# yangt1013/SPEINet

Hardware: AMD Instinct MI355X
Metric: deblurred 720p frames/sec (higher is better)
Workload: dtype f16 (correlation top2)

## Files before the change

include/speinet_hip.h:

```cpp
#ifndef SPEINET_HIP_H
#define SPEINET_HIP_H

#include <stdint.h>

#ifdef __cplusplus
extern "C" {
#endif

typedef void* spei_stream_t;

#define SPEI_ACT_NONE 0
#define SPEI_ACT_RELU 1
#define SPEI_ACT_GELU 2

#define SPEI_F32 0
#define SPEI_BF16 1
#define SPEI_F16 2

#define SPEI_CONV 0
#define SPEI_CONV_TRANSPOSED 1

int spei_version(void);
const char* spei_last_error(void);
const char* spei_arch(void);

int spei_any_nonzero(const float* x, int64_t n, int32_t* flag, spei_stream_t stream);

int spei_rl_prior(const float* img, float* out, float* scratch, int C, int H, int W, int iters, float lam,
                  spei_stream_t stream);

int spei_conv5_in(const float* img_chw, const float* w, const float* bias, float* out_hwc, int H, int W,
                  int Cout, spei_stream_t stream);

int spei_conv5_out(const float* in_hwc, int ldi, const float* w, const float* bias, float* out_chw, int H,
                   int W, int Cin, spei_stream_t stream);

int spei_igemm_f32(const float* a0, int lda0, int k0, const float* a1, int lda1, int k1, const float* w,
                   const float* bias, float* out, int ldo, const float* residual, int ldr,
                   const float* rowscale, int Hin, int Win, int Hout, int Wout, int N, int ksize, int stride,
                   int pad, int mode, int act, spei_stream_t stream);

int spei_igemm_f32_batched(const float* a0, int lda0, int k0, const float* a1, int lda1, int k1, const float* w,
                           const float* bias, float* out, int ldo, const float* residual, int ldr,
                           const float* rowscale, int Hin, int Win, int Hout, int Wout, int N, int ksize, int stride,
                           int pad, int mode, int act, int batch, spei_stream_t stream);

int spei_igemm_bf16(const float* a0, int lda0, int k0, const float* a1, int lda1, int k1, const void* w_hi,
                    const void* w_lo, const float* bias, float* out, int ldo, const float* residual, int ldr,
                    const float* rowscale, int Hin, int Win, int Hout, int Wout, int N, int ksize, int stride,
                    int pad, int mode, int act, spei_stream_t stream);

int spei_conv_slab16(int fmt, const void* a0, int lda0, int k0, const void* a1, int lda1, int k1, int a_fmt,
                     const void* wfrag_hi, const void* wfrag_lo, const float* bias, void* out, int ldo, int out_fmt,
                     const float* residual, int ldr, const float* rowscale, int Hin, int Win, int Hout, int Wout,
                     int N, int ksize, int stride, int pad, int act, int ln_input, spei_stream_t stream);

int spei_conv_slab16_batched(int fmt, const void* a0, int k0, int a_fmt, const void* wfrag, const void* wfrag_lo, const float* bias,
                             void* out, int out_fmt, const float* residual, int batch, int Hin, int Win, int Hout, int Wout, int N,
                             int ksize, int stride, int pad, int act, spei_stream_t stream);

int spei_conv_slab16_fa(int fmt, const float* x, int K, const void* x1, const float* s, const float* g1, const float* g2,
                        float* x_out, const void* wfrag, const float* bias, void* out, int ldo, int out_fmt, int H, int W, int N,
                        int ksize, int act, spei_stream_t stream);

int spei_conv32_ws16(int fmt, const void* a, int a_fmt, const void* wfrag, const float* bias, void* out, int out_fmt, int batch,
                     int H, int W, int act, spei_stream_t stream);

int spei_mlp_fused16(int fmt, const float* x, float* out, const void* w1_frag, const float* b1, const void* w2_frag,
                     const float* b2, int64_t M, spei_stream_t stream);

int spei_convt2_slab16(int fmt, const void* a0, int lda0, int k0, int a_fmt, const void* wfrag00, const void* wfrag01,
                       const void* wfrag10, const void* wfrag11, const float* bias, void* out, int ldo, int out_fmt,
                       int Hin, int Win, int N, int act, spei_stream_t stream);

int spei_convt2_slab16x3(const float* a0, int lda0, int k0, const void* const* whi4, const void* const* wlo4, const float* bias,
                         float* out, int ldo, int Hin, int Win, int N, int act, spei_stream_t stream);

int spei_conv3x3_256_pipe16(int fmt, const float* x, const void* w_frag, const float* bias, const float* residual, float* out,
                            int batch, int H, int W, spei_stream_t stream);

int spei_conv5_out_slab16(int fmt, const void* in, int ldi, int in_fmt, const void* wfrag, const float* bias32, float* out_chw,
                          int H, int W, spei_stream_t stream);

int spei_attn_fused16(int fmt, const float* x, float* out, const void* yhat, const void* wq_frag, const float* bq,
                      const void* wkv_frag, const float* bkv, const void* wproj_frag, const float* bproj,
                      const float* relbias, int H, int W, int shift, spei_stream_t stream);

int spei_attn_win4_16(int fmt, const float* x, float* out, const void* yhat, const void* wq_frag, const float* bq,
                      const void* wkv_frag, const float* bkv, const void* wproj_frag, const float* bproj,
                      const float* relbias, int batch, int H, int W, int shift, spei_stream_t stream);

int64_t spei_frame_post_ws_doubles(int H, int W, int border);
int spei_frame_post(const float* out_chw, const unsigned char* gt_hwc, unsigned char* out_hwc, int H, int W, int border,
                    double* ws, double* result, spei_stream_t stream);

int64_t spei_gate_ws_floats(int H, int W, int C);
int spei_resblock_gates(const void* x1, int x1_fmt, int H, int W, int C, const float* se_w1, const float* se_b1,
                        const float* se_w2, const float* se_b2, const float* cw_w, const float* cw_bn,
                        const float* hc_w, const float* hc_bn, float* s, float* g1, float* g2, float* ws,
                        spei_stream_t stream);
int spei_resblock_apply(const float* x, const void* x1, int x1_fmt, const float* s, const float* g1, const float* g2,
                        const float* extra, float* out, int ldo, int H, int W, int C, spei_stream_t stream);

int spei_resblock_gates_batched(const void* x1, int x1_fmt, int batch, int H, int W, int C, const float* se_w1, const float* se_b1,
                                const float* se_w2, const float* se_b2, const float* cw_w, const float* cw_bn, const float* hc_w,
                                const float* hc_bn, float* s, float* g1, float* g2, float* ws, spei_stream_t stream);
int spei_resblock_apply_batched(const float* x, const void* x1, int x1_fmt, const float* s, const float* g1, const float* g2, float* out,
                                int batch, int H, int W, int C, spei_stream_t stream);

int spei_layernorm256(const float* x, void* y, int out_fmt, const float* gamma, const float* beta, int64_t M,
                      spei_stream_t stream);

int spei_window_attention(const void* q, const void* kv, int io_fmt, const float* relbias, void* out, int H, int W,
                          int shift, spei_stream_t stream);
int spei_window_attention_batched(const void* q, const void* kv, int io_fmt, const float* relbias, void* out, int H, int W,
                                  int shift, int batch, spei_stream_t stream);

int spei_patch_invnorm(const float* f, int ldf, float* inv, int H, int W, int C, spei_stream_t stream);

int64_t spei_corr_ws_floats(int64_t n_lr);
int spei_corr_argmax(const float* lr, int ldl, const float* ref, int ldr, const float* inv_lr,
                     const float* inv_ref, int Hl, int Wl, int Hr, int Wr, int C, float* S, int32_t* arg,
                     float* ws, spei_stream_t stream);

int spei_split16(int fmt, const float* x, int ld, void* hi, void* lo, int64_t M, int C, spei_stream_t stream);
int spei_corr_argmax_bf16(const void* lr_hi, const void* lr_lo, const void* ref_hi, const void* ref_lo,
                          const float* inv_lr, const float* inv_ref, int Hl, int Wl, int Hr, int Wr, int C, float* S,
                          int32_t* arg, float* ws, spei_stream_t stream);

int spei_corr_slab16(int fmt, const void* lr_hi, const void* lr_lo, const void* ref_hi, const void* ref_lo,
                     const float* inv_lr, const float* inv_ref, int Hl, int Wl, int Hr, int Wr, int C, float* S,
                     int32_t* arg, float* ws, spei_stream_t stream);

int spei_corr_slab_top2_16(int fmt, const void* lr16, const void* ref16, const float* inv_lr, const float* inv_ref,
                           int Hl, int Wl, int Hr, int Wr, int C, float* S, int32_t* arg, float* S2, int32_t* arg2,
                           float* ws, spei_stream_t stream);
int64_t spei_corr_diag_ws_floats(int Hl, int Wl, int Hr, int Wr);
int spei_corr_diag_top2_16(int fmt, const void* lr16, const void* ref16, const float* inv_ref, int Hl, int Wl, int Hr, int Wr,
                           int C, float* S, int32_t* arg, float* S2, int32_t* arg2, float* ws, spei_stream_t stream);
int spei_corr_rescore(const float* lr, int ldl, const float* ref, int ldr, const float* inv_lr, const float* inv_ref,
                      int Hl, int Wl, int Hr, int Wr, int C, float* S, int32_t* arg, const float* S2, const int32_t* arg2,
                      spei_stream_t stream);

int spei_gather_fold(const float* ref, int ldr, const int32_t* arg, float* out, int ldo, int H3, int W3,
                     int Hr3, int Wr3, int C, int s, spei_stream_t stream);

int spei_rot90(const float* in, int ldi, float* out, int H, int W, int C, spei_stream_t stream);

// ... 91 lines not shown
```

speinet_amd/_lib.py:

```python
from __future__ import annotations

import ctypes as C
import os
import re

_HERE = os.path.dirname(os.path.abspath(__file__))
LIB_PATH = os.path.join(_HERE, "libspeinet_hip.so")
HEADER_PATH = os.path.join(os.path.dirname(_HERE), "include", "speinet_hip.h")

_lib = None

P = C.c_void_p
I = C.c_int
L = C.c_int64
F = C.c_float

SIGNATURES = {
    "spei_version": (I, []),
    "spei_last_error": (C.c_char_p, []),
    "spei_arch": (C.c_char_p, []),
    "spei_any_nonzero": (I, [P, L, P, P]),
    "spei_rl_prior": (I, [P, P, P, I, I, I, I, F, P]),
    "spei_conv5_in": (I, [P, P, P, P, I, I, I, P]),
    "spei_conv5_out": (I, [P, I, P, P, P, I, I, I, P]),
    "spei_igemm_f32": (I, [P, I, I, P, I, I, P, P, P, I, P, I, P, I, I, I, I, I, I, I, I, I, I, P]),
    "spei_igemm_f32_batched": (I, [P, I, I, P, I, I, P, P, P, I, P, I, P, I, I, I, I, I, I, I, I, I, I, I, P]),
    "spei_igemm_bf16": (I, [P, I, I, P, I, I, P, P, P, P, I, P, I, P, I, I, I, I, I, I, I, I, I, I, P]),
    "spei_conv_slab16": (I, [I, P, I, I, P, I, I, I, P, P, P, P, I, I, P, I, P, I, I, I, I, I, I, I, I, I, I, P]),
    "spei_conv32_ws16": (I, [I, P, I, P, P, P, I, I, I, I, I, P]),
    "spei_conv_slab16_fa": (I, [I, P, I, P, P, P, P, P, P, P, P, I, I, I, I, I, I, I, P]),
    "spei_attn_fused16": (I, [I, P, P, P, P, P, P, P, P, P, P, I, I, I, P]),
    "spei_attn_win4_16": (I, [I, P, P, P, P, P, P, P, P, P, P, I, I, I, I, P]),
    "spei_conv5_out_slab16": (I, [I, P, I, I, P, P, P, I, I, P]),
    "spei_convt2_slab16": (I, [I, P, I, I, I, P, P, P, P, P, P, I, I, I, I, I, I, P]),
    "spei_convt2_slab16x3": (I, [P, I, I, P, P, P, P, I, I, I, I, I, P]),
    "spei_conv3x3_256_pipe16": (I, [I, P, P, P, P, P, I, I, I, P]),
    "spei_mlp_fused16": (I, [I, P, P, P, P, P, P, L, P]),
    "spei_split16": (I, [I, P, I, P, P, L, I, P]),
    "spei_corr_slab16": (I, [I, P, P, P, P, P, P, I, I, I, I, I, P, P, P, P]),
    "spei_corr_slab_top2_16": (I, [I, P, P, P, P, I, I, I, I, I, P, P, P, P, P, P]),
    "spei_pack_split16": (I, [P, I, I, I, I, P, P, P]),
    "spei_corr_diag_ws_floats": (L, [I, I, I, I]),
    "spei_corr_diag_top2_16": (I, [I, P, P, P, I, I, I, I, I, P, P, P, P, P, P]),
    "spei_corr_rescore": (I, [P, I, P, I, P, P, I, I, I, I, I, P, P, P, P, P]),
    "spei_corr_argmax_bf16": (I, [P, P, P, P, P, P, I, I, I, I, I, P, P, P, P]),
    "spei_gate_ws_floats": (L, [I, I, I]),
    "spei_resblock_gates": (I, [P, I, I, I, I, P, P, P, P, P, P, P, P, P, P, P, P, P]),
    "spei_resblock_apply": (I, [P, P, I, P, P, P, P, P, I, I, I, I, P]),
    "spei_resblock_apply_batched": (I, [P, P, I, P, P, P, P, I, I, I, I, P]),
    "spei_resblock_gates_batched": (I, [P, I, I, I, I, I, P, P, P, P, P, P, P, P, P, P, P, P, P]),
    "spei_conv_slab16_batched": (I, [I, P, I, I, P, P, P, P, I, P, I, I, I, I, I, I, I, I, I, I, P]),
    "spei_layernorm256": (I, [P, P, I, P, P, L, P]),
    "spei_window_attention": (I, [P, P, I, P, P, I, I, I, P]),
    "spei_window_attention_batched": (I, [P, P, I, P, P, I, I, I, I, P]),
    "spei_patch_invnorm": (I, [P, I, P, I, I, I, P]),
    "spei_corr_ws_floats": (L, [L]),
    "spei_corr_argmax": (I, [P, I, P, I, P, P, I, I, I, I, I, P, P, P, P]),
    "spei_gather_fold": (I, [P, I, P, P, I, I, I, I, I, I, I, P]),
    "spei_rot90": (I, [P, I, P, I, I, I, P]),
    "spei_upsample_bicubic": (I, [P, I, P, I, I, I, I, I, I, P]),
    "spei_add": (I, [P, P, P, L, P]),
    "spei_wgrad_ws_floats": (L, [I, I, I, I, I]),
    "spei_conv_wgrad_f32_batched": (I, [P, I, P, I, P, P, P, I, I, I, I, I, I, I, I, I, I, P]),
    "spei_conv_wgrad_bf16x3_batched": (I, [P, I, P, I, P, P, P, I, I, I, I, I, I, I, I, I, I, P]),
    "spei_conv_wgrad_bf16_batched": (I, [P, I, P, I, P, P, P, I, I, I, I, I, I, I, I, I, I, P]),
    "spei_conv_s2_adjoint_slab16": (I, [P, I, P, P, I, I, I, I, I, P]),
    "spei_conv_wgrad_f32": (I, [P, I, P, I, P, P, P, I, I, I, I, I, I, I, I, I, P]),
    "spei_relu_bwd": (I, [P, P, P, L, P]),
    "spei_plane_ws_floats": (L, [I, I, I]),
    "spei_plane_stats": (I, [P, P, I, I, I, I, P, P, P, P, P, P, P]),
    "spei_plane_stats_batched": (I, [P, P, I, I, I, I, P, P, P, P, P, P, I, P]),
    "spei_resblock_apply_bwd": (I, [P, P, P, P, P, P, P, P, P, P, P, P, P, I, I, I, P]),
    "spei_resblock_apply_bwd_batched": (I, [P, P, P, P, P, P, P, P, P, P, P, P, P, I, I, I, I, P]),
    "spei_gate_train_saved_floats": (L, [I, I, I, I, I]),
    "spei_gate_train_ws_floats": (L, [I, I, I, I, I]),
    "spei_gate_train_nparams": (I, [I]),
    "spei_gate_maps_fwd": (I, [P, P, P, P, P, P, P, I, I, I, I, I, I, I, P, P, P, P, P, P]),
    "spei_gate_maps_bwd": (I, [P, P, P, P, P, P, P, I, I, I, I, I, I, P, P, P, P, P, P, P, P, P, P, P, P, P]),
    "spei_ln_bwd_blocks": (L, [L]),
    "spei_layernorm256_bwd": (I, [P, P, P, P, P, L, P]),
    "spei_gelu_fwd": (I, [P, P, L, P]),
    "spei_gelu_bwd": (I, [P, P, P, L, P]),
    "spei_window_attention_bwd": (I, [P, P, P, P, P, P, P, I, I, I, I, P]),
    "spei_window_attention16_train": (I, [P, P, P, P, I, I, I, I, P]),
    "spei_window_attention16_bwd": (I, [P, P, P, P, P, P, P, I, I, I, I, P]),
    "spei_scale_rows": (I, [P, P, P, L, I, P]),
    "spei_corr_s_bwd_lr": (I, [P, P, P, P, P, P, P, P, I, I, I, I, I, P]),
    "spei_search_bwd_ref": (I, [P, P, P, P, P, P, P, P, P, P, I, I, I, I, I, I, P]),
    "spei_upsample_bicubic_bwd": (I, [P, P, I, I, I, I, P]),
    "spei_rowdot": (I, [P, P, P, L, I, P]),
    "spei_frame_post_ws_doubles": (L, [I, I, I]),
    "spei_frame_post": (I, [P, P, P, I, I, I, P, P, P]),
    "spei_det_gray": (I, [P, P, I, I, I, P]),
    "spei_det_ws_floats": (L, [I, I, I, I]),
    "spei_det_features": (I, [P, P, P, I, I, I, I, P]),
}


def header_symbols() -> list:
    text = open(HEADER_PATH).read()
    text = re.sub(r"/\*.*?\*/", "", text, flags=re.S)
    return sorted(set(re.findall(r"\b(spei_[a-z0-9_]+)\s*\(", text)) - {"spei_stream_t"})


def lib():
    global _lib
    if _lib is None:
        if not os.path.exists(LIB_PATH):
            raise RuntimeError(
                f"{LIB_PATH} is missing: build it with `python -m speinet_amd.build` (hipcc --offload-arch=gfx950). "
                "speinet_amd has no CPU fallback.")
        import torch
# ... 13 lines not shown
```

speinet_amd/ops.py:

```python
from __future__ import annotations

import ctypes as C
from typing import Optional

import torch

from . import _lib
from .pack import BF16, F16, F32, LP_DTYPE, PackedW, fmt_of

ACT_NONE, ACT_RELU, ACT_GELU = 0, 1, 2
CONV, CONV_T = 0, 1

PRECISIONS = ("f32", "bf16x3", "bf16", "f16")
CORR_PRECISIONS = ("bf16x3", "single", "top2")
_CORR_ALIASES = {"bf16": "single", "bf16r": "top2", "f16": "single"}


class FMap:
    __slots__ = ("t", "H", "W", "C", "ld", "off")

    def __init__(self, t: torch.Tensor, H: int, W: int, C_: int, off: int = 0):
        assert t.is_cuda and t.dtype in (torch.float32, torch.bfloat16, torch.float16) and t.is_contiguous() and t.dim() == 2 and t.shape[0] == H * W
        self.t, self.H, self.W, self.C, self.ld, self.off = t, H, W, C_, t.shape[1], off
        assert off + C_ <= self.ld
# ... 87 lines not shown
    src, n = a[0], a[3]
    ks = a[4] if len(a) > 4 else k.get("ksize", 1)
    if n == 32 and src.C == 32 and ks == 5 and k.get("stride", a[5] if len(a) > 5 else 1) == 1:
        maps = getattr(src, "B", 1)
        return "level1", 2.0 * 25 * 32 * 32 * maps * src.H * src.W, _tensor_bytes(src) + _tensor_bytes(out)
    return "rest", 0.0, 0


def _family(name: str):
    def deco(fn):
        def wrapper(self, *a, **k):
            pr = self.profile
            if pr is None or "families" not in pr:
                return fn(self, *a, **k)
            st = torch.cuda.current_stream(self.device)
            s_, e_ = torch.cuda.Event(enable_timing=True), torch.cuda.Event(enable_timing=True)
            s_.record(st)
            out = fn(self, *a, **k)
            e_.record(st)
            pr["families"].setdefault(name, []).append((s_, e_))
            if name == "conv":
                sub, fl, by = _conv_sub(fn.__name__, a, k, out)
                rec = pr.setdefault("conv_sub", {}).setdefault(sub, {"events": [], "flops": 0.0, "bytes": 0})
                rec["events"].append((s_, e_))
                rec["flops"] += fl
                rec["bytes"] += by
            return out
        wrapper.__name__, wrapper.__doc__ = fn.__name__, fn.__doc__
        return wrapper
    return deco


def frame_post(out_chw: torch.Tensor, gt_hwc: torch.Tensor, border: int = 4):
    assert out_chw.is_cuda and out_chw.dtype == torch.float32 and out_chw.dim() == 3 and out_chw.shape[0] == 3 and out_chw.is_contiguous()
    h, w = out_chw.shape[1:]
    assert gt_hwc.shape == (h, w, 3) and gt_hwc.dtype == torch.uint8 and gt_hwc.device == out_chw.device and gt_hwc.is_contiguous()
    lib = _lib.lib()
    n = lib.spei_frame_post_ws_doubles(h, w, border)
    if n < 0:
        raise ValueError(f"frame {w}x{h} with border {border} is smaller than the 11x11 SSIM window")
    dev = out_chw.device
    u8 = torch.empty(h, w, 3, dtype=torch.uint8, device=dev)
    ws = torch.empty(n, dtype=torch.float64, device=dev)
    res = torch.empty(3, dtype=torch.float64, device=dev)
    with torch.cuda.device(dev):
        st = C.c_void_p(torch.cuda.current_stream(dev).cuda_stream)
        _lib.check(lib.spei_frame_post(_vp(out_chw.data_ptr()), _vp(gt_hwc.data_ptr()), _vp(u8.data_ptr()), h, w, border, _vp(ws.data_ptr()),
                                       _vp(res.data_ptr()), st), "spei_frame_post")
    return u8, res


CORR_DIAG_WS_MAX = 8 << 30


class CorrPlan:
    __slots__ = ("ctx", "s", "arg", "kernel", "main", "post", "keep")

    def __init__(self, ctx, s, arg, kernel, main, post, keep):
        self.ctx, self.s, self.arg, self.kernel, self.main, self.post, self.keep = ctx, s, arg, kernel, main, post, keep

    def launch(self, profile: Optional[dict] = None) -> None:
        ctx = self.ctx if profile is None else self.ctx.replace(profile=profile)
        st = ctx._stream()
        if ctx.profile is not None:
            ctx.profile["corr_kernel"] = self.kernel
        fam = ctx.profile is not None and "families" in ctx.profile
        if fam:
            f0, f1 = torch.cuda.Event(enable_timing=True), torch.cuda.Event(enable_timing=True)
            f0.record(torch.cuda.current_stream(ctx.device))
        with _timed(ctx, "corr_argmax"):
            for fn, name, args in self.main:
                _lib.check(fn(*args, st), name)
        for fn, name, args in self.post:
            _lib.check(fn(*args, st), name)
        if fam:
            f1.record(torch.cuda.current_stream(ctx.device))
            ctx.profile["families"].setdefault("correlation", []).append((f0, f1))


class Ctx:
    ACT_NONE, ACT_RELU, ACT_GELU = ACT_NONE, ACT_RELU, ACT_GELU
    CONV, CONV_T = CONV, CONV_T
    _FIELDS = ("precision", "corr_precision", "device", "use_slab", "bf16_storage", "x1_bf16", "fuse_mlp", "fuse_attn",
               "commute_upconv", "commute_any", "corr_bf16", "corr_diag", "fuse_apply", "split_decode", "batch_enc", "attn_win4", "conv32_ws", "conv3_pipe", "stage", "profile", "capture")
    SPLIT_STAGES = ("glue", "dec2")
    __slots__ = _FIELDS

    def __init__(self, precision: str = "f32", corr_precision: str = "bf16x3", device=None, use_slab: bool = True,
                 bf16_storage: bool = True, x1_bf16: bool = True, fuse_mlp: bool = True, fuse_attn: bool = True,
                 commute_upconv: bool = True, commute_any: bool = False, corr_bf16: bool = True,
                 corr_diag: bool = True, fuse_apply: bool = False, split_decode: bool = True, batch_enc: bool = True,
                 attn_win4: bool = True, conv32_ws: bool = True, conv3_pipe: bool = True, stage: Optional[dict] = None,
                 profile: Optional[dict] = None, capture: Optional[dict] = None):
        if precision not in PRECISIONS:
            raise ValueError(f"unknown precision {precision!r}")
        corr_precision = _CORR_ALIASES.get(corr_precision, corr_precision)
        if corr_precision not in CORR_PRECISIONS:
            raise ValueError(f"unknown correlation precision {corr_precision!r}")
        cur = torch.cuda.current_device() if torch.cuda.is_available() else 0
        device = torch.device("cuda", cur) if device is None else torch.device(device)
        if precision == "f16" and not use_slab:
            raise ValueError("the f16 mode is built on the slab kernels only")
        if device.type != "cuda":
            raise RuntimeError("speinet_amd runs on MI355X only (HIP kernels); there is no CPU path")
        if device.index is None:
            device = torch.device("cuda", cur)
        object.__setattr__(self, "precision", precision)
        object.__setattr__(self, "corr_precision", corr_precision)
        object.__setattr__(self, "device", device)
        for k, v in (("use_slab", use_slab), ("bf16_storage", bf16_storage), ("x1_bf16", x1_bf16), ("fuse_mlp", fuse_mlp),
                     ("fuse_attn", fuse_attn), ("commute_upconv", commute_upconv), ("commute_any", commute_any),
                     ("corr_bf16", corr_bf16), ("corr_diag", corr_diag), ("fuse_apply", fuse_apply), ("split_decode", split_decode), ("batch_enc", batch_enc), ("attn_win4", attn_win4), ("conv32_ws", conv32_ws), ("conv3_pipe", conv3_pipe)):
            object.__setattr__(self, k, bool(v))
        object.__setattr__(self, "stage", dict(stage) if stage else {})
        object.__setattr__(self, "profile", profile)
        object.__setattr__(self, "capture", capture)

    def __setattr__(self, k, v):
        raise AttributeError("Ctx is immutable; use replace()")

    def replace(self, **kw) -> "Ctx":
        d = {k: getattr(self, k) for k in self._FIELDS}
        d.update(kw)
        return Ctx(**d)

    def for_stage(self, name: str) -> "Ctx":
        o = self.stage.get(name)
        if o is None and self.split_decode and self.precision == "f16" and name in self.SPLIT_STAGES:
            o = {"precision": "bf16x3", "commute_any": True}
        return self.replace(**o) if o else self

    def _tp(self, t: Optional[torch.Tensor]) -> C.c_void_p:
        if t is None:
            return C.c_void_p(0)
        assert t.is_cuda and t.is_contiguous()
        assert t.device == self.device, f"tensor on {t.device}, call context on {self.device}"
        return C.c_void_p(t.data_ptr())

    def _fp(self, f: Optional[FMap]) -> C.c_void_p:
        if f is None:
            return C.c_void_p(0)
        assert f.t.device == self.device, f"feature map on {f.t.device}, call context on {self.device}"
        return C.c_void_p(f.ptr)

    def _stream(self) -> C.c_void_p:
        assert torch.cuda.current_device() == self.device.index, \
            f"current device cuda:{torch.cuda.current_device()} != call context {self.device}"
        return C.c_void_p(torch.cuda.current_stream(self.device).cuda_stream)

    @property
    def lp16(self) -> bool:
        return self.precision in ("bf16", "f16")

    @property
    def fmt(self) -> int:
        return F16 if self.precision == "f16" else BF16

    def inter_dtype(self) -> torch.dtype:
        return LP_DTYPE[self.fmt] if (self.lp16 and self.use_slab and self.bf16_storage) else torch.float32

    def any_nonzero(self, x: torch.Tensor, flag: torch.Tensor) -> None:
        _lib.check(_lib.lib().spei_any_nonzero(self._tp(x), x.numel(), self._tp(flag), self._stream()), "spei_any_nonzero")

    def rl_prior(self, img: torch.Tensor, iters: int, lam: float = 0.01) -> torch.Tensor:
        c, h, w = img.shape
        out = torch.empty_like(img)
        scratch = torch.empty_like(img)
        _lib.check(_lib.lib().spei_rl_prior(self._tp(img), self._tp(out), self._tp(scratch), c, h, w, iters, lam, self._stream()),
                   "spei_rl_prior")
        return out

    @_family("conv")
    def conv5_in(self, img: torch.Tensor, w: torch.Tensor, b: torch.Tensor, out: Optional[FMap] = None) -> FMap:
        c, h, wd = img.shape
        assert c == 3
        if out is None:
            out = FMap.empty(h, wd, b.numel(), img.device)
        assert (out.H, out.W, out.C, out.ld, out.off) == (h, wd, b.numel(), b.numel(), 0) and not out.lp
        _lib.check(_lib.lib().spei_conv5_in(self._tp(img), self._tp(w), self._tp(b), self._fp(out), h, wd, b.numel(), self._stream()),
                   "spei_conv5_in")
        return out

    @_family("conv")
    def conv5_out(self, f: FMap, w: torch.Tensor, b: torch.Tensor, out: torch.Tensor, w32=None,
                  b32: Optional[torch.Tensor] = None) -> torch.Tensor:
        assert out.shape == (3, f.H, f.W) and out.is_contiguous() and out.dtype == torch.float32
        if self.lp16 and self.use_slab and w32 is not None and f.C == 32:
            _lib.check(_lib.lib().spei_conv5_out_slab16(self.fmt, self._fp(f), f.ld, f.fmt, self._tp(w32.frag(self.fmt)), self._tp(b32),
                                                       self._tp(out), f.H, f.W, self._stream()), "spei_conv5_out_slab16")
            return out
        if f.lp:
            f = FMap(f.t.float(), f.H, f.W, f.C, f.off)
        _lib.check(_lib.lib().spei_conv5_out(self._fp(f), f.ld, self._tp(w), self._tp(b), self._tp(out), f.H, f.W, f.C, self._stream()),
                   "spei_conv5_out")
        return out

    def _conv3_pipe_ok(self, a, w, N: int, ksize: int, stride: int, act: int, residual, out) -> bool:
        return (self.conv3_pipe and self.lp16 and self.use_slab and ksize == 3 and stride == 1 and N == 256 and a.C == 256 and act == ACT_NONE
                and a.H % 6 == 0 and a.W % 16 == 0 and a.H * a.W <= (1 << 21) and a.t.dtype == torch.float32 and getattr(a, "ld", 256) == 256
                and getattr(a, "off", 0) == 0 and getattr(w, "fhi", None) is not None and tuple(w.shape) == (9, 256, 256)
                and (out is None or (out.t.dtype == torch.float32 and getattr(out, "ld", 256) == 256 and getattr(out, "off", 0) == 0
                                     and out.t.data_ptr() != a.t.data_ptr()))
                and (residual is None or (residual.t.dtype == torch.float32 and getattr(residual, "ld", 256) == 256 and getattr(residual, "off", 0) == 0)))

    @_family("conv")
    def igemm(self, a0: FMap, w, bias: Optional[torch.Tensor], N: int, ksize: int = 1, stride: int = 1,
              mode: int = CONV, act: int = ACT_NONE, a1: Optional[FMap] = None, residual: Optional[FMap] = None,
              rowscale: Optional[torch.Tensor] = None, out: Optional[FMap] = None, out_dtype=torch.float32,
              ln_input: bool = False) -> FMap:
        prec = self.precision
        pad = ksize // 2
        if mode == CONV:
            ho, wo = (a0.H + 2 * pad - ksize) // stride + 1, (a0.W + 2 * pad - ksize) // stride + 1
        else:
            ho, wo = a0.H * stride, a0.W * stride
        if out is None:
            out = FMap.empty(ho, wo, N, a0.t.device, out_dtype)
        assert out.H == ho and out.W == wo and out.C == N
        k0, k1 = a0.C, (a1.C if a1 is not None else 0)
        slab = prec != "f32" and self.use_slab and mode == CONV
        assert slab or (mode == CONV_T and self.lp16 and self.use_slab) or not (a0.lp or out.lp), \
            "16-bit activations are only supported by the slab kernel"
        assert a1 is None or a1.t.dtype == a0.t.dtype
        assert residual is None or not residual.lp
        assert all(f.t.dtype in (torch.float32, LP_DTYPE[self.fmt]) for f in (a0, out)), "16-bit tensors must be in the mode's format"
        if torch.is_tensor(w):
            w = PackedW(w, a0.t.device)
        assert not ln_input or (slab and w.fhi is not None), "ln_input is a feature of the slab kernel"
        assert tuple(w.shape) == (ksize * ksize, N, k0 + k1), (tuple(w.shape), ksize, N, k0, k1)
        if a1 is not None:
            assert (a1.H, a1.W) == (a0.H, a0.W)
        if residual is not None:
            assert (residual.H, residual.W, residual.C) == (ho, wo, N)
        if rowscale is not None:
            assert rowscale.numel() == ho * wo
        tp, fp = self._tp, self._fp
        common = (fp(out), out.ld, fp(residual), residual.ld if residual is not None else 0, tp(rowscale), a0.H, a0.W, ho, wo, N,
                  ksize, stride, pad, mode, act, self._stream())
        srcs = (fp(a0), a0.ld, k0, fp(a1), a1.ld if a1 is not None else 0, k1)
        lib = _lib.lib()
        if (mode == CONV and a1 is None and rowscale is None and not ln_input and out_dtype == torch.float32
                and self._conv3_pipe_ok(a0, w, N, ksize, stride, act, residual, out)):
            _lib.check(lib.spei_conv3x3_256_pipe16(self.fmt, fp(a0), tp(w.frag(self.fmt)), tp(bias), fp(residual), fp(out), 1, a0.H, a0.W,
                                                   self._stream()), "spei_conv3x3_256_pipe16")
        elif (self.conv32_ws_available() and mode == CONV and ksize == 5 and stride == 1 and k0 == 32 and N == 32 and a1 is None
                and residual is None and rowscale is None and not ln_input and act in (ACT_NONE, ACT_RELU) and w.fhi is not None
                and (a0.ld, a0.off, out.ld, out.off) == (32, 0, 32, 0) and a0.t.data_ptr() != out.t.data_ptr()):
            _lib.check(lib.spei_conv32_ws16(self.fmt, fp(a0), a0.fmt, tp(w.frag(self.fmt)), tp(bias), fp(out), out.fmt, 1, a0.H, a0.W, act,
                                            self._stream()), "spei_conv32_ws16")
        elif (mode == CONV_T and self.lp16 and self.use_slab and ksize == 3 and stride == 2 and a1 is None and residual is None
                and rowscale is None and N % 32 == 0 and k0 % 32 == 0):
            cf = w.convT_class_frags(self.fmt)
            _lib.check(lib.spei_convt2_slab16(self.fmt, fp(a0), a0.ld, k0, a0.fmt, tp(cf[(0, 0)]), tp(cf[(0, 1)]), tp(cf[(1, 0)]),
                                              tp(cf[(1, 1)]), tp(bias), fp(out), out.ld, out.fmt, a0.H, a0.W, N, act,
                                              self._stream()), "spei_convt2_slab16")
        elif (mode == CONV_T and prec == "bf16x3" and self.use_slab and ksize == 3 and stride == 2 and a1 is None and residual is None
                and rowscale is None and N % 32 == 0 and k0 % 32 == 0 and not a0.lp and not out.lp):
            _hi, _lo, ph, pl = w.convT_class_frags_split()
            _lib.check(lib.spei_convt2_slab16x3(fp(a0), a0.ld, k0, ph, pl, tp(bias), fp(out), out.ld, a0.H, a0.W, N, act, self._stream()),
                       "spei_convt2_slab16x3")
        elif prec == "f32":
            _lib.check(lib.spei_igemm_f32(*srcs, tp(w.f32), tp(bias), *common), "spei_igemm_f32")
        elif slab and w.fhi is not None:
            dims = (a0.H * a0.W, 1, ho * wo, 1) if (ksize == 1 and stride == 1) else (a0.H, a0.W, ho, wo)
            _lib.check(lib.spei_conv_slab16(
                self.fmt, *srcs, a0.fmt, tp(w.frag(self.fmt)), tp(w.flo) if prec == "bf16x3" else _vp(0), tp(bias), fp(out), out.ld,
                out.fmt, fp(residual), residual.ld if residual is not None else 0,
                tp(rowscale), *dims, N, ksize, stride, pad, act, int(ln_input), self._stream()), "spei_conv_slab16")
        else:
            assert prec != "f16", "f16: N and K must be multiples of 32 (slab kernel)"
            _lib.check(lib.spei_igemm_bf16(*srcs, tp(w.hi), tp(w.lo) if prec == "bf16x3" else _vp(0), tp(bias), *common),
                       "spei_igemm_bf16")
        return out

    def linear(self, x: torch.Tensor, w, b: Optional[torch.Tensor], act: int = ACT_NONE,
               residual: Optional[torch.Tensor] = None, out: Optional[torch.Tensor] = None, out_dtype=torch.float32,
               ln_input: bool = False) -> torch.Tensor:
        m, k = x.shape
        if torch.is_tensor(w):
            w = PackedW(w.reshape(1, *w.shape), x.device)
        n = w.shape[1]
        if out is None:
            out = torch.empty(m, n, device=x.device, dtype=out_dtype)
        self.igemm(FMap(x, m, 1, k), w, b, n, act=act, ln_input=ln_input,
                   residual=FMap(residual, m, 1, n) if residual is not None else None, out=FMap(out, m, 1, n))
        return out

    @_family("streaming")
    def resblock_gates(self, x1: FMap, pk: dict):
        dev = x1.t.device
        lib = _lib.lib()
        tp = self._tp
        assert x1.off == 0 and x1.ld == x1.C
        s = torch.empty(x1.C, device=dev)
        g1 = torch.empty(x1.H, x1.C, device=dev)
        g2 = torch.empty(x1.W, x1.C, device=dev)
        ws = torch.empty(lib.spei_gate_ws_floats(x1.H, x1.W, x1.C), device=dev)
        _lib.check(lib.spei_resblock_gates(self._fp(x1), x1.fmt, x1.H, x1.W, x1.C, tp(pk["se_w1"]), tp(pk["se_b1"]), tp(pk["se_w2"]),
                                           tp(pk["se_b2"]), tp(pk["cw_w"]), tp(pk["cw_bn"]), tp(pk["hc_w"]), tp(pk["hc_bn"]),
                                           tp(s), tp(g1), tp(g2), tp(ws), self._stream()), "spei_resblock_gates")
        return s, g1, g2

    def apply_fused_available(self, c: int) -> bool:
        return self.lp16 and self.use_slab and self.x1_bf16 and self.fuse_apply and c in (32, 64, 128, 256)

    def resblock(self, x, pk: dict, extra: Optional[FMap] = None, out: Optional[FMap] = None, defer: bool = False):
        idt = self.inter_dtype()
        if isinstance(x, tuple):
            px, px1, ps, pg1, pg2 = x
            c = px.C
            xn = FMap.empty(px.H, px.W, c, px.t.device)
            t = FMap.empty(px.H, px.W, c, px.t.device, idt)
            w1 = pk["w1"] if not torch.is_tensor(pk["w1"]) else PackedW(pk["w1"], px.t.device)
            _lib.check(_lib.lib().spei_conv_slab16_fa(self.fmt, self._fp(px), c, self._fp(px1), self._tp(ps), self._tp(pg1), self._tp(pg2),
                                                      self._fp(xn), self._tp(w1.frag(self.fmt)), self._tp(pk["b1"]), self._fp(t), t.ld, t.fmt,
                                                      px.H, px.W, c, 5, ACT_RELU, self._stream()), "spei_conv_slab16_fa")
            x = xn
        else:
            c = x.C
            assert x.off == 0 and x.ld == c
            t = self.igemm(x, pk["w1"], pk["b1"], c, ksize=5, act=ACT_RELU, out_dtype=idt)
        x1 = self.igemm(t, pk["w2"], pk["b2"], c, ksize=5, out_dtype=idt if self.x1_bf16 else torch.float32)
        s, g1, g2 = self.resblock_gates(x1, pk)
        if defer:
            return (x, x1, s, g1, g2)
        if out is None:
            out = FMap.empty(x.H, x.W, c, x.t.device)
        if extra is not None:
            assert extra.off == 0 and extra.ld == c
        self._apply(x, x1, s, g1, g2, extra, out, c)
        return out

    @_family("streaming")
    def _apply(self, x, x1, s, g1, g2, extra, out, c):
        _lib.check(_lib.lib().spei_resblock_apply(self._fp(x), self._fp(x1), x1.fmt, self._tp(s), self._tp(g1), self._tp(g2),
                                                  self._fp(extra), self._fp(out), out.ld, x.H, x.W, c, self._stream()),
                   "spei_resblock_apply")

    def batched_available(self) -> bool:
        return self.batched_kernels() and self.x1_bf16 and self.bf16_storage and not self.fuse_apply and self.batch_enc

    def conv32_ws_available(self) -> bool:
        return self.lp16 and self.use_slab and self.conv32_ws

    def batched_kernels(self) -> bool:
        return self.lp16 and self.use_slab

    @_family("conv")
    def igemm_batched(self, a: BMap, w, bias: torch.Tensor, N: int, ksize: int, stride: int = 1, act: int = ACT_NONE,
                      out_dtype=torch.float32, residual: Optional[BMap] = None, out: Optional[BMap] = None) -> BMap:
        assert self.batched_kernels() and not torch.is_tensor(w) and w.fhi is not None
        pad = ksize // 2
        ho, wo = (a.H + 2 * pad - ksize) // stride + 1, (a.W + 2 * pad - ksize) // stride + 1
        assert tuple(w.shape) == (ksize * ksize, N, a.C) and a.t.dtype in (torch.float32, LP_DTYPE[self.fmt])
        if out is None:
            out = BMap.empty(a.B, ho, wo, N, a.t.device, out_dtype)
        assert (out.B, out.H, out.W, out.C) == (a.B, ho, wo, N) and out.t.data_ptr() != a.t.data_ptr()
        if residual is not None:
            assert (residual.B, residual.H, residual.W, residual.C) == (a.B, ho, wo, N) and residual.t.dtype == torch.float32
            assert residual.t.data_ptr() != a.t.data_ptr()
        tp = self._tp
        if out_dtype == torch.float32 and self._conv3_pipe_ok(a, w, N, ksize, stride, act, residual, out):
            _lib.check(_lib.lib().spei_conv3x3_256_pipe16(self.fmt, tp(a.t), tp(w.frag(self.fmt)), tp(bias),
                                                          tp(residual.t) if residual is not None else _vp(0), tp(out.t), a.B, a.H, a.W,
                                                          self._stream()), "spei_conv3x3_256_pipe16")
            return out
        if (self.conv32_ws_available() and ksize == 5 and stride == 1 and a.C == 32 and N == 32 and residual is None
                and act in (ACT_NONE, ACT_RELU)):
            _lib.check(_lib.lib().spei_conv32_ws16(self.fmt, tp(a.t), a.fmt, tp(w.frag(self.fmt)), tp(bias), tp(out.t), out.fmt, a.B, a.H, a.W,
                                                   act, self._stream()), "spei_conv32_ws16")
            return out
        _lib.check(_lib.lib().spei_conv_slab16_batched(self.fmt, tp(a.t), a.C, a.fmt, tp(w.frag(self.fmt)), _vp(0), tp(bias), tp(out.t), out.fmt,
                                                       tp(residual.t) if residual is not None else _vp(0), a.B, a.H, a.W, ho, wo, N, ksize,
                                                       stride, pad, act, self._stream()),
                   "spei_conv_slab16_batched")
        return out

    def resblock_batched(self, x: BMap, pk: dict) -> BMap:
        idt = self.inter_dtype()
        c, dev = x.C, x.t.device
        lib = _lib.lib()
        tp = self._tp
        t = self.igemm_batched(x, pk["w1"], pk["b1"], c, 5, act=ACT_RELU, out_dtype=idt)
        x1 = self.igemm_batched(t, pk["w2"], pk["b2"], c, 5, out_dtype=idt)
        del t
        return self._gates_apply_batched(x, x1, pk)

    @_family("streaming")
    def _gates_apply_batched(self, x: BMap, x1: BMap, pk: dict) -> BMap:
        c, dev = x.C, x.t.device
        lib = _lib.lib()
        tp = self._tp
        s = torch.empty(x.B, c, device=dev)
        g1 = torch.empty(x.B, x.H, c, device=dev)
        g2 = torch.empty(x.B, x.W, c, device=dev)
        ws = torch.empty(x.B * lib.spei_gate_ws_floats(x.H, x.W, c), device=dev)
        _lib.check(lib.spei_resblock_gates_batched(tp(x1.t), x1.fmt, x.B, x.H, x.W, c, tp(pk["se_w1"]), tp(pk["se_b1"]), tp(pk["se_w2"]),
                                                   tp(pk["se_b2"]), tp(pk["cw_w"]), tp(pk["cw_bn"]), tp(pk["hc_w"]), tp(pk["hc_bn"]),
                                                   tp(s), tp(g1), tp(g2), tp(ws), self._stream()), "spei_resblock_gates_batched")
        out = BMap.empty(x.B, x.H, x.W, c, dev)
        _lib.check(lib.spei_resblock_apply_batched(tp(x.t), tp(x1.t), x1.fmt, tp(s), tp(g1), tp(g2), tp(out.t), x.B, x.H, x.W, c,
                                                   self._stream()), "spei_resblock_apply_batched")
        return out

    def ln_fused_available(self) -> bool:
        return self.precision != "f32" and self.use_slab

    def attn_fused_available(self) -> bool:
        return self.lp16 and self.use_slab and self.fuse_attn and self.bf16_storage

    def mlp_fused_available(self) -> bool:
        return self.lp16 and self.use_slab and self.fuse_mlp

    def swin_multi_available(self) -> bool:
        return self.attn_fused_available() and self.attn_win4 and self.mlp_fused_available() and self.batched_kernels()

    @_family("swin")
    def attn_fused(self, x: torch.Tensor, yhat: torch.Tensor, bk: dict, H: int, W: int, shift: int, out: torch.Tensor) -> torch.Tensor:
        assert x.shape[0] % (H * W) == 0 and x.shape[1] == 256 and x.dtype == torch.float32 and out.shape == x.shape and out.dtype == torch.float32
        f = self.fmt
        assert yhat.shape == x.shape and yhat.dtype == LP_DTYPE[f]
        tp = self._tp
        batch = x.shape[0] // (H * W)
        if self.attn_win4:
            _lib.check(_lib.lib().spei_attn_win4_16(f, tp(x), tp(out), tp(yhat), tp(bk["wq"].frag(f)), tp(bk["bq"]), tp(bk["wkv"].frag(f)),
                                                    tp(bk["bkv"]), tp(bk["wproj"].frag(f)), tp(bk["bproj"]), tp(bk["relbias"]), batch, H, W,
                                                    shift, self._stream()), "spei_attn_win4_16")
            return out
        assert batch == 1, "the two-window kernel takes one map per launch"
        _lib.check(_lib.lib().spei_attn_fused16(f, tp(x), tp(out), tp(yhat), tp(bk["wq"].frag(f)), tp(bk["bq"]), tp(bk["wkv"].frag(f)),
                                                tp(bk["bkv"]), tp(bk["wproj"].frag(f)), tp(bk["bproj"]), tp(bk["relbias"]), H, W, shift,
                                                self._stream()), "spei_attn_fused16")
        return out

    @_family("swin")
    def mlp_fused(self, x: torch.Tensor, w1, b1: torch.Tensor, w2, b2: torch.Tensor, out: torch.Tensor) -> torch.Tensor:
        assert x.shape[1] == 256 and x.dtype == torch.float32 and out.shape == x.shape and out.dtype == torch.float32
        assert tuple(w1.shape) == (1, 512, 256) and tuple(w2.shape) == (1, 256, 512)
        tp = self._tp
        f = self.fmt
        _lib.check(_lib.lib().spei_mlp_fused16(f, tp(x), tp(out), tp(w1.frag(f)), tp(b1), tp(w2.frag(f)), tp(b2), x.shape[0], self._stream()),
                   "spei_mlp_fused16")
        return out

    def layernorm(self, x: torch.Tensor, g: Optional[torch.Tensor] = None, b: Optional[torch.Tensor] = None,
                  out: Optional[torch.Tensor] = None, out_dtype=torch.float32) -> torch.Tensor:
        assert x.shape[1] == 256 and x.is_contiguous() and x.dtype == torch.float32
        if out is None:
            out = torch.empty(x.shape, device=x.device, dtype=out_dtype)
        tp = self._tp
        _lib.check(_lib.lib().spei_layernorm256(tp(x), tp(out), fmt_of(out.dtype), tp(g), tp(b), x.shape[0], self._stream()),
                   "spei_layernorm256")
        return out
# ... 102 lines not shown
```

Baseline: 40.33.

## Add weight-stationary persistent 5x5 conv kernel for 64-channel layers

Adds a persistent kernel for 5x5 stride-1 convolutions with 64 input and 64 output channels. Each block keeps its whole weight slice in registers, double-buffers input tiles in LDS so the next tile's global loads overlap the current tile's MFMAs, and splits the reduction across wave pairs, combining the halves through LDS. It is routed in for 64-channel resblock convs in both the single-map and batched paths, on by default through the conv32_ws flag. The cost is very high register pressure with one block per CU, plus extra LDS exchange traffic.

Result: faster. 41.18 (median of 6 runs) (+2.1%).

```diff
diff --git a/include/speinet_hip.h b/include/speinet_hip.h
--- a/include/speinet_hip.h
+++ b/include/speinet_hip.h
@@ -64,6 +64,9 @@
                         int ksize, int act, spei_stream_t stream);
 
 int spei_conv32_ws16(int fmt, const void* a, int a_fmt, const void* wfrag, const float* bias, void* out, int out_fmt, int batch,
+                     int H, int W, int act, spei_stream_t stream);
+
+int spei_conv64_ws16(int fmt, const void* a, int a_fmt, const void* wfrag, const float* bias, void* out, int out_fmt, int batch,
                      int H, int W, int act, spei_stream_t stream);
 
 int spei_mlp_fused16(int fmt, const float* x, float* out, const void* w1_frag, const float* b1, const void* w2_frag,
diff --git a/speinet_amd/_lib.py b/speinet_amd/_lib.py
--- a/speinet_amd/_lib.py
+++ b/speinet_amd/_lib.py
@@ -28,6 +28,7 @@
     "spei_igemm_bf16": (I, [P, I, I, P, I, I, P, P, P, P, I, P, I, P, I, I, I, I, I, I, I, I, I, I, P]),
     "spei_conv_slab16": (I, [I, P, I, I, P, I, I, I, P, P, P, P, I, I, P, I, P, I, I, I, I, I, I, I, I, I, I, P]),
     "spei_conv32_ws16": (I, [I, P, I, P, P, P, I, I, I, I, I, P]),
+    "spei_conv64_ws16": (I, [I, P, I, P, P, P, I, I, I, I, I, P]),
     "spei_conv_slab16_fa": (I, [I, P, I, P, P, P, P, P, P, P, P, I, I, I, I, I, I, I, P]),
     "spei_attn_fused16": (I, [I, P, P, P, P, P, P, P, P, P, P, I, I, I, P]),
     "spei_attn_win4_16": (I, [I, P, P, P, P, P, P, P, P, P, P, I, I, I, I, P]),
diff --git a/speinet_amd/csrc/conv64_ws16.hip b/speinet_amd/csrc/conv64_ws16.hip
--- /dev/null
+++ b/speinet_amd/csrc/conv64_ws16.hip
@@ -0,0 +1,289 @@
+#include "common.h"
+
+namespace {
+
+constexpr int C = 64, KS = 5, PAD = 2, NTAP = KS * KS;
+constexpr int TH = 6, TW = 32;
+constexpr int IH = TH + KS - 1, IW = TW + KS - 1;
+constexpr int PITCH = 2 * C + 16;
+constexpr int SLAB = IH * IW * PITCH;
+constexpr int NTHR = 256;
+constexpr int HR = TH / 2;
+constexpr int XCH_WAVE = HR * 4 * 64 * 16;
+constexpr int LDS_BYTES = 2 * SLAB + 4 * XCH_WAVE;
+constexpr int PF = 1;
+
+struct WsParams {
+    const void* a;
+    const void* wfrag;
+    const float* bias;
+    void* out;
+    int H, W, batch, act;
+    int tiles_x, tiles_y, total;
+    long long* stamps;
+};
+
+__device__ __forceinline__ void mfma_aw(f32x16& acc, const lpv<_Float16>::x8& w, const lpv<_Float16>::x8& b) {
+    asm volatile("v_mfma_f32_32x32x16_f16 %0, %1, %2, %0" : "+v"(acc) : "a"(w), "v"(b));
+}
+__device__ __forceinline__ void mfma_aw(f32x16& acc, const lpv<__bf16>::x8& w, const lpv<__bf16>::x8& b) {
+    asm volatile("v_mfma_f32_32x32x16_bf16 %0, %1, %2, %0" : "+v"(acc) : "a"(w), "v"(b));
+}
+__device__ __forceinline__ void mfma_aw0(f32x16& acc, const lpv<_Float16>::x8& w, const lpv<_Float16>::x8& b) {
+    asm volatile("v_mfma_f32_32x32x16_f16 %0, %1, %2, 0" : "=v"(acc) : "a"(w), "v"(b));
+}
+__device__ __forceinline__ void mfma_aw0(f32x16& acc, const lpv<__bf16>::x8& w, const lpv<__bf16>::x8& b) {
+    asm volatile("v_mfma_f32_32x32x16_bf16 %0, %1, %2, 0" : "=v"(acc) : "a"(w), "v"(b));
+}
+
+template <typename TA> struct Chunk { static constexpr int CPP = sizeof(TA) == 4 ? 16 : 8; };
+
+template <typename LP, typename TA, typename TO>
+__global__ __launch_bounds__(NTHR, 1) void conv64_ws_kernel(const WsParams p) {
+    typedef typename lpv<LP>::x8 lp8;
+    typedef typename lpv<LP>::x4 lp4;
+    constexpr int CPP = Chunk<TA>::CPP;
+    constexpr int NCH = IH * IW * CPP;
+    constexpr int NIT = (NCH + NTHR - 1) / NTHR;
+    constexpr int NPH = sizeof(TA) == 4 ? 3 : 1;
+    constexpr int NITH = (NIT + NPH - 1) / NPH;
+    constexpr int PSTEP = 2 * NTAP / NPH;
+    static_assert(NPH == 1 || NPH == 3, "the MFMA loop below is cut for one or three staging parts");
+    extern __shared__ __attribute__((aligned(16))) unsigned char smem[];
+
+    const int tid = threadIdx.x, lane = tid & 63, wave = tid >> 6;
+    const int fr = lane & 31, fk = lane >> 5;
+    const int nt = wave >> 1, kh = wave & 1;
+
+    lp8 wreg[NTAP][2];
+    {
+        const LP* wp = static_cast<const LP*>(p.wfrag) + ((size_t)nt * NTAP * 4 + 2 * kh) * 512 + lane * 8;
+#pragma unroll
+        for (int t = 0; t < NTAP; ++t)
+#pragma unroll
+            for (int s = 0; s < 2; ++s) wreg[t][s] = *reinterpret_cast<const lp8*>(wp + (t * 4 + s) * 512);
+    }
+    float biasv[16];
+#pragma unroll
+    for (int r = 0; r < 16; ++r) biasv[r] = p.bias ? p.bias[32 * nt + 8 * (r >> 2) + 4 * fk + (r & 3)] : 0.f;
+
+    typedef u32x4 stage_t;
+    stage_t sreg[NITH];
+    const size_t map_elems = (size_t)p.H * p.W * C;
+    const int per_map = p.tiles_x * p.tiles_y;
+    const int G = gridDim.x;
+    const int slot = (G & 7) ? (int)blockIdx.x : (int)(blockIdx.x & 7) * (G >> 3) + (int)(blockIdx.x >> 3);
+    auto tile_of = [&](int t) {
+        const int base = t - (int)blockIdx.x;
+        return base + G <= p.total ? base + slot : t;
+    };
+    auto tile_origin = [&](int t, int& b, int& oy0, int& ox0) {
+        t = tile_of(t);
+        b = t / per_map;
+        const int r = t - b * per_map;
+        const int ty = r / p.tiles_x;
+        oy0 = ty * TH;
+        ox0 = (r - ty * p.tiles_x) * TW;
+    };
+    constexpr int PPI = NTHR / CPP, E = 16 / (int)sizeof(TA);
+    const int p0 = tid / CPP, sub = tid - p0 * CPP;
+    const int iy0 = p0 / IW, ix0 = p0 - iy0 * IW;
+    const int lds0 = p0 * PITCH + sub * (sizeof(TA) == 4 ? 8 : 16);
+    auto advance = [](int& iy, int& ix) {
+        ix += PPI % IW;
+        iy += PPI / IW;
+        if (ix >= IW) { ix -= IW; ++iy; }
+    };
+    auto load_slab = [&](int t, int ph) {
+        int b, oy0, ox0;
+        tile_origin(t, b, oy0, ox0);
+        const TA* base = static_cast<const TA*>(p.a) + (size_t)b * map_elems + sub * E;
+        int iy = iy0, ix = ix0;
+#pragma unroll
+        for (int it = 0; it < NIT; ++it) {
+            if (it >= ph * NITH && it < (ph + 1) * NITH) {
+                const int iyc = min(iy, IH - 1);
+                const int gy = min(max(oy0 - PAD + iyc, 0), p.H - 1), gx = min(max(ox0 - PAD + ix, 0), p.W - 1);
+                sreg[it - ph * NITH] = *reinterpret_cast<const stage_t*>(base + ((size_t)gy * p.W + gx) * C);
+            }
+            advance(iy, ix);
+        }
+    };
+    auto store_slab = [&](int t, int buf, int ph, int lo, int hi) {
+        int b, oy0, ox0;
+        tile_origin(t, b, oy0, ox0);
+        unsigned char* sl = smem + buf * SLAB + lds0;
+        int iy = iy0, ix = ix0;
+#pragma unroll
+        for (int it = 0; it < NIT; ++it) {
+            if (it >= ph * NITH + lo && it < ph * NITH + hi && it < (ph + 1) * NITH && iy < IH) {
+                const int j = it - ph * NITH;
+                const bool ok = ((unsigned)(oy0 - PAD + iy) < (unsigned)p.H) & ((unsigned)(ox0 - PAD + ix) < (unsigned)p.W);
+                if constexpr (sizeof(TA) == 4) {
+                    const f32x4 v = __builtin_bit_cast(f32x4, sreg[j]);
+                    lp4 h = to_lp4<LP>(v);
+                    if (!ok) h = lp4{(LP)0.f, (LP)0.f, (LP)0.f, (LP)0.f};
+                    *reinterpret_cast<lp4*>(sl + it * PPI * PITCH) = h;
+                } else {
+                    *reinterpret_cast<stage_t*>(sl + it * PPI * PITCH) = ok ? sreg[j] : stage_t{0u, 0u, 0u, 0u};
+                }
+            }
+            advance(iy, ix);
+        }
+    };
+
+    int t = blockIdx.x;
+    if (t >= p.total) return;
+#pragma unroll
+    for (int ph = 0; ph < NPH; ++ph) {
+        load_slab(t, ph);
+        store_slab(t, 0, ph, 0, NITH);
+    }
+    lds_barrier();
+
+    int boff[TH];
+#pragma unroll
+    for (int i = 0; i < TH; ++i) boff[i] = (((i + HR * kh) % TH) * IW + fr) * PITCH + kh * 64 + fk * 16;
+    unsigned char* const xch = smem + 2 * SLAB;
+
+    int buf = 0;
+    for (; t < p.total; t += gridDim.x, buf ^= 1) {
+        const int tn = t + gridDim.x;
+        const bool more = tn < p.total;
+        const int tl = more ? tn : t;
+        const bool st_ = t == (int)blockIdx.x + (int)gridDim.x;
+        if (st_) SPEI_STAMP(p.stamps, 0);
+        load_slab(tl, 0);
+        if (st_) SPEI_STAMP(p.stamps, 1);
+        __builtin_amdgcn_sched_barrier(0);
+
+        const unsigned char* sl = smem + buf * SLAB;
+        f32x16 acc[TH];
+        lp8 bq[PF + 1][TH];
+        auto step_off = [](int step) { const int tap = step >> 1; return ((tap / KS) * IW + (tap % KS)) * PITCH + (step & 1) * 32; };
+#pragma unroll
+        for (int d = 0; d < PF; ++d)
+#pragma unroll
+            for (int i = 0; i < TH; ++i) bq[d][i] = *reinterpret_cast<const lp8*>(sl + boff[i] + step_off(d));
+        auto steps = [&](auto lo_c, auto hi_c) {
+            constexpr int LO = decltype(lo_c)::value, HI = decltype(hi_c)::value;
+#pragma unroll
+            for (int step = LO; step < HI; ++step) {
+                const int tap = step >> 1, s2 = step & 1;
+                if (step + PF < NTAP * 2) {
+#pragma unroll
+                    for (int i = 0; i < TH; ++i)
+                        bq[(step + PF) % (PF + 1)][i] = *reinterpret_cast<const lp8*>(sl + boff[i] + step_off(step + PF));
+                }
+#pragma unroll
+                for (int i = 0; i < TH; ++i) {
+                    if (step == 0) mfma_aw0(acc[i], wreg[tap][s2], bq[step % (PF + 1)][i]);
+                    else mfma_aw(acc[i], wreg[tap][s2], bq[step % (PF + 1)][i]);
+                }
+                if (NPH == 1 && step >= NTAP && ((step - NTAP) & 1) == 0 && (step - NTAP) / 2 < NITH)
+                    store_slab(tl, buf ^ 1, 0, (step - NTAP) / 2, (step - NTAP) / 2 + 1);
+            }
+        };
+        if constexpr (NPH == 1) {
+            steps(std::integral_constant<int, 0>{}, std::integral_constant<int, 2 * NTAP>{});
+        } else {
+            steps(std::integral_constant<int, 0>{}, std::integral_constant<int, PSTEP>{});
+            store_slab(tl, buf ^ 1, 0, 0, NITH);
+            load_slab(tl, 1);
+            steps(std::integral_constant<int, PSTEP>{}, std::integral_constant<int, 2 * PSTEP>{});
+            store_slab(tl, buf ^ 1, 1, 0, NITH);
+            load_slab(tl, 2);
+            steps(std::integral_constant<int, 2 * PSTEP>{}, std::integral_constant<int, 2 * NTAP>{});
+        }
+
+        __builtin_amdgcn_sched_barrier(0);
+        asm volatile("s_nop 7\n\ts_nop 7\n\ts_nop 7" ::: "memory");
+        __builtin_amdgcn_sched_barrier(0);
+        if (st_) SPEI_STAMP(p.stamps, 2);
+        {
+            f32x4* x = reinterpret_cast<f32x4*>(xch + wave * XCH_WAVE) + lane;
+#pragma unroll
+            for (int j = 0; j < HR; ++j)
+#pragma unroll
+                for (int g = 0; g < 4; ++g)
+                    x[(j * 4 + g) * 64] = f32x4{acc[HR + j][4 * g], acc[HR + j][4 * g + 1], acc[HR + j][4 * g + 2], acc[HR + j][4 * g + 3]};
+        }
+        lds_barrier();
+        if (st_) SPEI_STAMP(p.stamps, 3);
+        {
+            int b, oy0, ox0;
+            tile_origin(t, b, oy0, ox0);
+            TO* ob = static_cast<TO*>(p.out) + (size_t)b * map_elems;
+            const int ox = ox0 + fr;
+            const f32x4* x = reinterpret_cast<const f32x4*>(xch + (wave ^ 1) * XCH_WAVE) + lane;
+#pragma unroll
+            for (int j = 0; j < HR; ++j) {
+                const int oy = oy0 + kh * HR + j;
+                if (oy < p.H && ox < p.W) {
+                    TO* o = ob + ((size_t)oy * p.W + ox) * C + 32 * nt + 4 * fk;
+#pragma unroll
+                    for (int g = 0; g < 4; ++g) {
+                        const f32x4 q = x[(j * 4 + g) * 64];
+                        f32x4 v;
+#pragma unroll
+                        for (int e = 0; e < 4; ++e) {
+                            v[e] = acc[j][4 * g + e] + q[e] + biasv[4 * g + e];
+                            if (p.act == SPEI_ACT_RELU) v[e] = fmaxf(v[e], 0.f);
+                        }
+                        if constexpr (sizeof(TO) == 4) *reinterpret_cast<f32x4*>(o + 8 * g) = v;
+                        else *reinterpret_cast<lp4*>(o + 8 * g) = to_lp4<LP>(v);
+                    }
+                }
+            }
+        }
+        if (st_) SPEI_STAMP(p.stamps, 4);
+        if (NPH > 1) store_slab(tl, buf ^ 1, NPH - 1, 0, NITH);
+        else store_slab(tl, buf ^ 1, 0, (NTAP + 1) / 2, NITH);
+        lds_barrier();
+        if (st_) SPEI_STAMP(p.stamps, 5);
+    }
+}
+
+template <typename LP>
+int launch_ws(const WsParams& p, int a16, int o16, hipStream_t st) {
+    const size_t lds = LDS_BYTES;
+    const int cus = spei_num_cus();
+    const dim3 grid(p.total < cus ? p.total : cus);
+    if (a16 && o16) {
+        ensure_dyn_lds<&conv64_ws_kernel<LP, LP, LP>>(lds);
+        hipLaunchKernelGGL((conv64_ws_kernel<LP, LP, LP>), grid, dim3(NTHR), lds, st, p);
+    } else if (!a16 && o16) {
+        ensure_dyn_lds<&conv64_ws_kernel<LP, float, LP>>(lds);
+        hipLaunchKernelGGL((conv64_ws_kernel<LP, float, LP>), grid, dim3(NTHR), lds, st, p);
+    } else if (a16 && !o16) {
+        ensure_dyn_lds<&conv64_ws_kernel<LP, LP, float>>(lds);
+        hipLaunchKernelGGL((conv64_ws_kernel<LP, LP, float>), grid, dim3(NTHR), lds, st, p);
+    } else {
+        ensure_dyn_lds<&conv64_ws_kernel<LP, float, float>>(lds);
+        hipLaunchKernelGGL((conv64_ws_kernel<LP, float, float>), grid, dim3(NTHR), lds, st, p);
+    }
+    return 0;
+}
+
+}
+
+extern "C" int spei_conv64_ws16(int fmt, const void* a, int a_fmt, const void* wfrag, const float* bias, void* out, int out_fmt, int batch,
+                                int H, int W, int act, spei_stream_t stream) {
+    SPEI_REQUIRE(a && wfrag && out, "spei_conv64_ws16: null pointer");
+    SPEI_REQUIRE((fmt == SPEI_BF16 || fmt == SPEI_F16) && (a_fmt == SPEI_F32 || a_fmt == fmt) && (out_fmt == SPEI_F32 || out_fmt == fmt),
+                 "spei_conv64_ws16: fmt=%d a_fmt=%d out_fmt=%d", fmt, a_fmt, out_fmt);
+    SPEI_REQUIRE(batch >= 1 && H > 0 && W > 0 && (int64_t)batch * cdiv(H, TH) * cdiv(W, TW) < (1ll << 30) && (int64_t)H * W < (1ll << 26),
+                 "spei_conv64_ws16: batch=%d of %dx%d", batch, H, W);
+    SPEI_REQUIRE(act == SPEI_ACT_NONE || act == SPEI_ACT_RELU, "spei_conv64_ws16: act=%d", act);
+    SPEI_REQUIRE(((uintptr_t)a | (uintptr_t)wfrag | (uintptr_t)out) % 16 == 0 && a != out, "spei_conv64_ws16: 16-byte alignment, out must not be the input");
+    WsParams p;
+    p.a = a; p.wfrag = wfrag; p.bias = bias; p.out = out; p.H = H; p.W = W; p.batch = batch; p.act = act;
+    p.tiles_x = cdiv(W, TW); p.tiles_y = cdiv(H, TH); p.total = batch * p.tiles_x * p.tiles_y;
+    p.stamps = spei_stamp_buffer();
+    hipStream_t st = (hipStream_t)stream;
+    const int a16 = a_fmt != SPEI_F32, o16 = out_fmt != SPEI_F32;
+    const int rc = fmt == SPEI_F16 ? launch_ws<_Float16>(p, a16, o16, st) : launch_ws<__bf16>(p, a16, o16, st);
+    if (rc) return rc;
+    SPEI_CHECK_LAUNCH("spei_conv64_ws16");
+    return 0;
+}
diff --git a/speinet_amd/ops.py b/speinet_amd/ops.py
--- a/speinet_amd/ops.py
+++ b/speinet_amd/ops.py
@@ -193,7 +193,7 @@
     ACT_NONE, ACT_RELU, ACT_GELU = ACT_NONE, ACT_RELU, ACT_GELU
     CONV, CONV_T = CONV, CONV_T
     _FIELDS = ("precision", "corr_precision", "device", "use_slab", "bf16_storage", "x1_bf16", "fuse_mlp", "fuse_attn",
-               "commute_upconv", "commute_any", "corr_bf16", "corr_diag", "fuse_apply", "split_decode", "batch_enc", "attn_win4", "conv32_ws", "conv3_pipe", "stage", "profile", "capture")
+               "commute_upconv", "commute_any", "corr_bf16", "corr_diag", "fuse_apply", "split_decode", "batch_enc", "attn_win4", "conv32_ws", "conv64_ws", "conv3_pipe", "stage", "profile", "capture")
     SPLIT_STAGES = ("glue", "dec2")
     __slots__ = _FIELDS
 
@@ -201,7 +201,8 @@
                  bf16_storage: bool = True, x1_bf16: bool = True, fuse_mlp: bool = True, fuse_attn: bool = True,
                  commute_upconv: bool = True, commute_any: bool = False, corr_bf16: bool = True,
                  corr_diag: bool = True, fuse_apply: bool = False, split_decode: bool = True, batch_enc: bool = True,
-                 attn_win4: bool = True, conv32_ws: bool = True, conv3_pipe: bool = True, stage: Optional[dict] = None,
+                 attn_win4: bool = True, conv32_ws: bool = True, conv64_ws: Optional[bool] = None, conv3_pipe: bool = True,
+                 stage: Optional[dict] = None,
                  profile: Optional[dict] = None, capture: Optional[dict] = None):
         if precision not in PRECISIONS:
             raise ValueError(f"unknown precision {precision!r}")
@@ -223,6 +224,7 @@
                      ("fuse_attn", fuse_attn), ("commute_upconv", commute_upconv), ("commute_any", commute_any),
                      ("corr_bf16", corr_bf16), ("corr_diag", corr_diag), ("fuse_apply", fuse_apply), ("split_decode", split_decode), ("batch_enc", batch_enc), ("attn_win4", attn_win4), ("conv32_ws", conv32_ws), ("conv3_pipe", conv3_pipe)):
             object.__setattr__(self, k, bool(v))
+        object.__setattr__(self, "conv64_ws", None if conv64_ws is None else bool(conv64_ws))
         object.__setattr__(self, "stage", dict(stage) if stage else {})
         object.__setattr__(self, "profile", profile)
         object.__setattr__(self, "capture", capture)
@@ -359,6 +361,11 @@
                 and (a0.ld, a0.off, out.ld, out.off) == (32, 0, 32, 0) and a0.t.data_ptr() != out.t.data_ptr()):
             _lib.check(lib.spei_conv32_ws16(self.fmt, fp(a0), a0.fmt, tp(w.frag(self.fmt)), tp(bias), fp(out), out.fmt, 1, a0.H, a0.W, act,
                                             self._stream()), "spei_conv32_ws16")
+        elif (self.conv64_ws_available() and mode == CONV and ksize == 5 and stride == 1 and k0 == 64 and N == 64 and a1 is None
+                and residual is None and rowscale is None and not ln_input and act in (ACT_NONE, ACT_RELU) and w.fhi is not None
+                and (a0.ld, a0.off, out.ld, out.off) == (64, 0, 64, 0) and a0.t.data_ptr() != out.t.data_ptr()):
+            _lib.check(lib.spei_conv64_ws16(self.fmt, fp(a0), a0.fmt, tp(w.frag(self.fmt)), tp(bias), fp(out), out.fmt, 1, a0.H, a0.W, act,
+                                            self._stream()), "spei_conv64_ws16")
         elif (mode == CONV_T and self.lp16 and self.use_slab and ksize == 3 and stride == 2 and a1 is None and residual is None
                 and rowscale is None and N % 32 == 0 and k0 % 32 == 0):
             cf = w.convT_class_frags(self.fmt)
@@ -454,6 +461,9 @@
     def conv32_ws_available(self) -> bool:
         return self.lp16 and self.use_slab and self.conv32_ws
 
+    def conv64_ws_available(self) -> bool:
+        return self.lp16 and self.use_slab and (self.conv32_ws if self.conv64_ws is None else self.conv64_ws)
+
     def batched_kernels(self) -> bool:
         return self.lp16 and self.use_slab
 
@@ -480,6 +490,11 @@
                 and act in (ACT_NONE, ACT_RELU)):
             _lib.check(_lib.lib().spei_conv32_ws16(self.fmt, tp(a.t), a.fmt, tp(w.frag(self.fmt)), tp(bias), tp(out.t), out.fmt, a.B, a.H, a.W,
                                                    act, self._stream()), "spei_conv32_ws16")
+            return out
+        if (self.conv64_ws_available() and ksize == 5 and stride == 1 and a.C == 64 and N == 64 and residual is None
+                and act in (ACT_NONE, ACT_RELU)):
+            _lib.check(_lib.lib().spei_conv64_ws16(self.fmt, tp(a.t), a.fmt, tp(w.frag(self.fmt)), tp(bias), tp(out.t), out.fmt, a.B, a.H, a.W,
+                                                   act, self._stream()), "spei_conv64_ws16")
             return out
         _lib.check(_lib.lib().spei_conv_slab16_batched(self.fmt, tp(a.t), a.C, a.fmt, tp(w.frag(self.fmt)), _vp(0), tp(bias), tp(out.t), out.fmt,
                                                        tp(residual.t) if residual is not None else _vp(0), a.B, a.H, a.W, ho, wo, N, ksize,
```
